# limuhit/360-Image-Compression

Hardware: AMD Instinct MI355X
Metric: ERP Mpixels/s enc+dec @512x1024 model-idx 3; bitstream bit-exact vs ref (higher is better)
Workload: dtype f32; 1 GPU; 192/GPU synthetic 512x1024 ERPs, model-idx 3 --ssim seed, latent+importance bitstreams, entropy enc+dec; streams=3, masks=smooth

## Files before the change

360-image-compression_amd/csrc/cconv4v6_dc.inc:

```
#define D6_GRID 256
#define D6_TAPE_BLOCKS 16
#define D6_TAPE_WAVES 6
#define D3_S0 (4 + C4_PS - 1)
#define D3_C0 2
#define D3_SP(h, w) ((h) + (w) - 1 + 2 * D3_S0)
#define D3_HP(h) ((h) + 2 * D3_C0)
struct Dc3Args {
    const float *x, *packed, *bias, *act, *residual;
    float *out;
    int ngroup, cout, hidden, H, W, npb, x_mod, N, psum, n_gb, n_gbv, nseg, pack0, gstep;
    int wblk;
    int nprod;
    int tape_c, tape_n, tape_total;
    unsigned tape_magic;
    unsigned tape_nw4[2];
};
struct Dc3Packed {
    const float *x, *packed, *bias, *act, *residual;
    float *out;
    unsigned w0;
    unsigned hw;
    int npb, x_mod, N;
    unsigned pg;
    int wblk, tape_n, tape_total;
// ... 38 lines not shown
        out[nwin++] = (unsigned)k | (unsigned)slo << 3 | (unsigned)shi << 9 | (unsigned)a0 << 15 | 1u << 21;
        pos = ((a0 + (shi - slo) + 4) / 4 + 1) * 4;
        slo = shi + 1;
        if (slo > hi) { slo = lo; ++k; }
    }
    return nwin;
}
__host__ __device__ __forceinline__ void dc6_wave_start(unsigned word, int lo, int hi, int h, int c, int wv, int &k, int &slo) {
    k = 0; slo = lo;
    if (wv == 0) return;
    const unsigned st = (word >> (9 * ((wv - 1) >> 1))) & 511u;
    k = st & 7; slo = st >> 3;
    if (!(wv & 1)) {
        unsigned pc[3];
        dc6_wave_pieces(lo, hi, h, c, k, slo, pc);
    }
}
#ifndef D6_STAGE_AT_END
#define D6_STAGE_AT_END 1
#endif
#ifndef D6_NB
#define D6_NB 2
#endif
#define D6_COLS 68
#define D6_QPR (D6_COLS / 4)
#define D6_ROWS (9 + C4_PS - 1)
#define D6_XQ(CIN) (4 * D6_ROWS * D6_QPR)
#define D6_XFL(CIN) (D6_XQ(CIN) * 4)

#define DPP_WAVE_SHL1 0x130
#define DPP_WAVE_SHR1 0x138
__device__ __forceinline__ float dpp_shl1(float v) {
    return __builtin_bit_cast(float, __builtin_amdgcn_update_dpp(0, __builtin_bit_cast(int, v), DPP_WAVE_SHL1, 0xf, 0xf, true));
}
__device__ __forceinline__ float dpp_shr1(float v) {
    return __builtin_bit_cast(float, __builtin_amdgcn_update_dpp(0, __builtin_bit_cast(int, v), DPP_WAVE_SHR1, 0xf, 0xf, true));
}

template <int CIN, int CLS, int XPLANE>
__device__ __forceinline__ void conv6_load(float *r0, const float *xl) {
    static_for<9>([&](auto dd) {
        constexpr int d = decltype(dd)::value, gid = CIN == 4 ? ((CLS - d) & 3) : 0, kmin = d > 4 ? d - 4 : 0, kmax = d < 4 ? d : 4;
        constexpr int k0 = kmax < 2 ? kmax : (kmin > 2 ? kmin : 2);
        if constexpr (CIN == 4 || (d & 3) == CLS) r0[d] = xl[gid * XPLANE + d * D6_COLS + k0];
    });
}
template <int CIN, int CLS, int D_LO, int D_HI>
__device__ __forceinline__ void conv6_diags(f32x4 *acc, const float *r0, float w0, float w1) {
    static_for<9>([&](auto dd) {
        constexpr int d = decltype(dd)::value, kmin = d > 4 ? d - 4 : 0, kmax = d < 4 ? d : 4;
        if constexpr (d >= D_LO && d <= D_HI && (CIN == 4 || (d & 3) == CLS)) {
            static_for<kmax - kmin + 1>([&](auto kk) {
                constexpr int kh = kmin + decltype(kk)::value, tap = 5 * kh + (d - kh), i = CIN == 4 ? tap : (tap - CLS) / 4;
                acc[i] = mfma4<i % 16>(i < 16 ? w0 : w1, r0[d], acc[i]);
            });
        }
    });
    __builtin_amdgcn_sched_barrier(0);
}
template <int CIN, int CLS>
__device__ __forceinline__ void conv6_align(f32x4 *acc) {
    static_for<9>([&](auto dd) {
        constexpr int d = decltype(dd)::value, kmin = d > 4 ? d - 4 : 0, kmax = d < 4 ? d : 4;
        constexpr int k0 = kmax < 2 ? kmax : (kmin > 2 ? kmin : 2);
        if constexpr (CIN == 4 || (d & 3) == CLS) {
            static_for<kmax - kmin + 1>([&](auto kk) {
                constexpr int kh = kmin + decltype(kk)::value, tap = 5 * kh + (d - kh), i = CIN == 4 ? tap : (tap - CLS) / 4, sh = kh - k0;
                static_for<(sh > 0 ? sh : -sh)>([&](auto) {
#pragma unroll
                    for (int r = 0; r < 4; ++r) acc[i][r] = sh > 0 ? dpp_shl1(acc[i][r]) : dpp_shr1(acc[i][r]);
                });
            });
        }
    });
}

struct W8 {
    float a0, a1, a2, a3, b0, b1, b2, b3;
    template <int H, int J> __device__ __forceinline__ float get() const {
        if constexpr (H == 0) return J == 0 ? a0 : (J == 1 ? a1 : (J == 2 ? a2 : a3));
        else return J == 0 ? b0 : (J == 1 ? b1 : (J == 2 ? b2 : b3));
    }
};

#define D6_SEG_STEP 60
#define D6_NSEG(h) ((h) <= 64 ? 1 : 1 + ((h) - 62 + D6_SEG_STEP - 1) / D6_SEG_STEP)
#ifdef DC6_STAMP
__device__ unsigned long long dc6_stamps[256 * 12 * 10];
#ifndef DC6_STAMP_CIN
#define DC6_STAMP_CIN 4
#endif
#define DC6_T(i) do { if constexpr (CIN == DC6_STAMP_CIN && !SEG) { const unsigned long long t_ = __builtin_amdgcn_s_memtime(); st[i] += t_ - t0; t0 = t_; } } while (0)
LIC360_API int lic360_dc6_stamps(unsigned long long *host_out, int clear) {
    if (host_out) HIP_TRY(hipMemcpyFromSymbol(host_out, HIP_SYMBOL(dc6_stamps), sizeof(dc6_stamps)));
    if (clear) { static unsigned long long z[256 * 12 * 10]; HIP_TRY(hipMemcpyToSymbol(HIP_SYMBOL(dc6_stamps), z, sizeof(z))); }
    return 0;
}
#else
#define DC6_T(i)
#endif
template <int CIN, int CLS, bool SEG, bool LAT = false, bool TAPE = false, bool LIST = false>
__device__ __forceinline__ void dc6_body(const Dc3Args &a, const Dc3Tape *tape, const uint4 *__restrict__ list, const int *__restrict__ lcnt, float *xs, float *comb,
                                         int (*trec)[16], int tid, int lane, int ps) {
    static_assert(!LIST || (TAPE && !SEG && !LAT), "list launches are throughput-mode launches of images of at most 64 rows");
    constexpr int XQ = D6_XQ(CIN), XFL = D6_XFL(CIN);
    static_assert(XQ <= C4_THREADS, "one quad slot per thread");
    constexpr int XPLANE = D6_ROWS * D6_COLS;
    const int H = a.H, W = a.W, G = a.ngroup, S = H + W - 1, HP = D3_HP(H);
    const int gs = a.gstep;
    constexpr int TCS = CIN == 1 ? 4 : 1;
    const long SKP = (long)D3_SP(H, W) * HP, tcs = 4 * SKP;
    f32x4 acc[NAcc<CIN>::value];
#ifdef DC6_STAMP
    unsigned long long st[10] = {0, 0, 0, 0, 0, 0, 0, 0, 0, 0}, t0 = __builtin_amdgcn_s_memtime();
    const unsigned long long t_entry = t0;
#endif
    const bool flat = gs == 1;
    const int xcd = flat ? 0 : blockIdx.x & 7, xstep = flat ? 1 : 8, wg_in_xcd = flat ? blockIdx.x : blockIdx.x >> 3;
    const int wgs_per_xcd = flat ? D6_GRID : (D6_GRID - xcd + 7) >> 3;
    auto nth_task = [&](int k) __attribute__((always_inline)) { return k * wgs_per_xcd + ((k & 1) ? wgs_per_xcd - 1 - wg_in_xcd : wg_in_xcd); };
    const int ns_x = flat ? a.N : (a.N - xcd + 7) >> 3;
    const int nseg = SEG ? a.nseg : 1;
    constexpr bool PACK = true;
    const bool pack_last = PACK && SEG && a.pack0 != 0;
    const int per_j = SEG ? ns_x * (nseg - 1) + (pack_last ? (ns_x + 1) >> 1 : ns_x) : 0;
    const int tape_c = TAPE ? a.tape_c : 0;
    const unsigned nw4[2] = {a.tape_nw4[0], a.tape_nw4[1]};
    auto blk_tasks = [&](int j) __attribute__((always_inline)) {
        return tape_c ? a.tape_n * (int)((nw4[(j >> 3) & 1] >> ((j & 7) * 4)) & 15u) : ns_x;
    };
    uint4 lrec = make_uint4(0u, 0u, 0u, 0u);
    if constexpr (LIST) {
        if (CLS == 0 && ps == 0) {
            int u = nth_task(lane);
            if (u > a.tape_total - 1) u = a.tape_total - 1;
            lrec = list[(long)xcd * a.tape_total + u];
        }
    }
    int n_my_ = 0;
    if constexpr (LIST) n_my_ = __builtin_amdgcn_readfirstlane(lcnt[xcd]);
    else if constexpr (SEG) n_my_ = per_j * a.n_gbv;
    else if (tape_c) n_my_ = a.tape_total;
    else n_my_ = ns_x * a.n_gbv;
    const int n_my = n_my_;
    int pk = -1, pq = 0;
    auto decode = [&](int u, int &g0, int &n, int &s0, int &seg, int &nb2, int &prb, int &packed) __attribute__((always_inline)) {
        nb2 = -1; prb = 0; packed = 0;
        if constexpr (LIST) {
            uint4 r;
            if (pk < 64) {
                r.x = (unsigned)__builtin_amdgcn_readlane((int)lrec.x, pk); r.y = (unsigned)__builtin_amdgcn_readlane((int)lrec.y, pk);
                r.z = (unsigned)__builtin_amdgcn_readlane((int)lrec.z, pk); r.w = (unsigned)__builtin_amdgcn_readlane((int)lrec.w, pk);
            } else r = list[(long)xcd * a.tape_total + u];
            g0 = (int)(r.x & 127u);
            n = (int)(r.x >> 10);
            s0 = a.psum - g0;
            seg = 0;
            if ((r.x >> 7) & 7u) { seg = (int)(r.y & 0x3fffffu); nb2 = (int)r.z; prb = (int)r.w; packed = 4; }
            packed |= (int)((r.y >> 22) & 7u) << 4;
        } else if constexpr (!SEG) {
            int j = 0, rem = u;
            for (; j < a.n_gbv - 1 && rem >= blk_tasks(j); ++j) rem -= blk_tasks(j);
            g0 = (a.n_gb - 1 - j) * gs;
            s0 = a.psum - g0;
            seg = 0;
            if (tape_c && (int)((nw4[(j >> 3) & 1] >> ((j & 7) * 4)) & 15u) < tape_c) {
                const int wv = a.tape_n == 1 ? rem : (int)__umulhi((unsigned)rem, a.tape_magic), tp = rem - wv * a.tape_n;
                n = xcd + 8 * tp * tape_c;
                int lo = 1 << 30, hi = -1;
#pragma unroll
                for (int q = 0; q < C4_PS; ++q) {
                    const int sq = s0 - q, l = sq >= W ? sq - W + 1 : 0, h2 = sq < H ? sq : H - 1;
                    if (g0 + q < G && sq >= 0 && sq < S) { lo = l < lo ? l : lo; hi = h2 > hi ? h2 : hi; }
                }
                int k, slo;
                dc6_wave_start(tape->s[j & (D6_TAPE_BLOCKS - 1)], lo, hi, H, tape_c, wv, k, slo);
                unsigned pc[3];
                dc6_wave_pieces(lo, hi, H, tape_c, k, slo, pc);
                seg = (int)pc[0]; nb2 = (int)pc[1]; prb = (int)pc[2];
                packed = 4;
            } else n = xcd + xstep * rem;
        } else {
            const int j = u / per_j, rem = u - j * per_j;
            g0 = (a.n_gb - 1 - j) * gs;
            s0 = a.psum - g0;
            if (pack_last && rem >= ns_x * (nseg - 1)) {
                seg = nseg - 1;
                n = xcd + 16 * (rem - ns_x * (nseg - 1));
                nb2 = n + 8;
                prb = H - 28;
                packed = 2;
            } else {
                seg = rem / ns_x;
                n = xcd + xstep * (rem - seg * ns_x);
            }
// ... 51 lines not shown
    auto issue_setup = [&]() __attribute__((always_inline)) {
        const int ig0 = rec(iq, 1), n = rec(iq, 2), is0 = rec(iq, 3), iseg = rec(iq, 4), inb = rec(iq, 5), iprb = rec(iq, 6);
        const int ipacked = rec(iq, 7) & 15;
        iL = steps_of(ig0);
        irl = ig0 + (C4_PS - 1) + 4 + a.hidden;
        const int irb = ipacked == 4 ? 0 : ((SEG && !ipacked) ? D6_SEG_STEP * iseg : iprb);
        ixn = (const char *)(a.x + (long)(n % a.x_mod) * G * CIN * SKP + (long)is0 * HP + irb);
        {
            const int qc = qa % D6_QPR;
            if (TAPE && ipacked == 4) {
                unsigned sh = 0u;
                bool cov = false;
                const unsigned stride8 = (unsigned)(8 * G * CIN * SKP * 4);
#pragma unroll
                for (int wi = 0; wi < 3; ++wi) {
                    const unsigned wd = (unsigned)(wi == 0 ? iseg : (wi == 1 ? inb : iprb));
                    const int k = wd & 7, slo = (wd >> 3) & 63, shi = (wd >> 9) & 63, a0 = (wd >> 15) & 63;
                    const bool in = (wd >> 21) != 0 && 4 * qc + 3 >= a0 && 4 * qc <= a0 + (shi - slo) + 4;
                    if (in) { sh = (unsigned)k * stride8 + (unsigned)((slo - a0) * 4); cov = true; }
                }
                t_off = cov ? offA + sh : 0u;
                t_off0 = cov ? offA0 + sh : 0u;
            } else if (SEG && PACK && ipacked) {
                const bool hb = qc > 8;
                const unsigned shift = hb ? (unsigned)(((long)((inb >= 0 ? inb : n) % a.x_mod) - (long)(n % a.x_mod)) * G * CIN * SKP * 4 - 9 * 16) : 0u;
                t_off = offA + shift;
                t_off0 = offA0 + shift;
            } else {
                const int lo = is0 - (gs - 1) - W + 1 - irb, hi = (is0 < H - 1 ? is0 : H - 1) - irb;
                const bool col_ok = qc >= ((lo > 0 ? lo : 0) >> 2) && qc <= ((hi + 4) >> 2);
                t_off = col_ok ? offA : 0u;
                t_off0 = col_ok ? offA0 : 0u;
            }
        }
        const int gg = ig0 + ps < G ? ig0 + ps : G - 1;
        iwp = (const char *)(a.packed + (((long)(n / a.npb) * G + gg) * a.wblk) * 1024);
    };
    if (!ivalid) return;
    issue_setup();
    const long tcs_b = tcs * 4;
    constexpr int WPSTEP = CIN == 4 ? 4096 : 8192;
    const char *px = ixn, *pw = iwp;
    auto issue_x2 = [&](f32x4 &ra, f32x4 &rb, int &tc0) __attribute__((always_inline)) -> const char * {
        const char *pwr = pw;
        tc0 = itc;
        unsigned oa, ob;
        if constexpr (CIN == 4) {
            oa = rowA < irl - itc ? t_off : t_off0;
            ob = rowA < irl - itc - 1 ? t_off : t_off0;
        } else {
            const int ta = itc + tcoA, tb = ta + TCS;
            oa = rowA < irl - ta ? t_off : t_off0;
            ob = rowA < irl - tb ? t_off : t_off0;
            if (ta >= G) oa = offP0;
            if (tb >= G) ob = offP0;
        }
        ra = *(const f32x4 *)(px + oa);
        rb = *(const f32x4 *)(px + (itc + TCS < G ? tcs_b : 0) + ob);
        if (ivalid) {
            px += 2 * tcs_b;
            pw += WPSTEP;
            itc += 2 * TCS;
            if (itc >= iL) {
                itc = 0;
                ++iq;
                ivalid = rec(iq, 0) != 0;
                if (ivalid) { issue_setup(); px = ixn; pw = iwp; }
                else { px -= 2 * tcs_b; pw -= WPSTEP; itc = tc0; }
            }
        }
        return pwr;
    };
    auto issue_w2 = [&](const char *p, int tc0, W8 &w) __attribute__((always_inline)) {
        (void)tc0;
        const f32x4 v = *(const f32x4 *)(p + offW);
        w.a0 = v[0]; w.a1 = v[1];
        if constexpr (CIN == 4) { w.b0 = v[2]; w.b1 = v[3]; }
        else {
            const f32x4 u = *(const f32x4 *)(p + offW + 4096);
            w.a2 = v[2]; w.a3 = v[3];
            w.b0 = u[0]; w.b1 = u[1]; w.b2 = u[2]; w.b3 = u[3];
        }
    };
    constexpr bool MIDST = D6_STAGE_AT_END == 0 || CIN == 1 || LAT || LIST;
    constexpr int NB = D6_NB, NBUF = 2 * D6_NB;
    static_assert(NB == 1 || NB == 2, "one or two double steps per barrier");
    f32x4 xa0 = {0.f, 0.f, 0.f, 0.f}, xb0 = xa0, xa1 = xa0, xb1 = xa0;
    W8 w0, w1;
    int tcw;
    { const char *p = issue_x2(xa0, xb0, tcw); issue_w2(p, tcw, w0); }
    { const char *p = issue_x2(xa1, xb1, tcw); issue_w2(p, tcw, w1); }
    if (hasA) { *(f32x4 *)ldsA = xa0; *(f32x4 *)(ldsA + XFL) = xb0; }
    int tcw_next, tcw_next2 = 0;
    const char *pw_next = issue_x2(xa0, xb0, tcw_next), *pw_next2 = nullptr;
    if constexpr (NB == 2) {
        if (hasA) { *(f32x4 *)(ldsA + 2 * XFL) = xa1; *(f32x4 *)(ldsA + 3 * XFL) = xb1; }
        pw_next2 = issue_x2(xa1, xb1, tcw_next2);
    }
    const f32x4 zero4 = {0.f, 0.f, 0.f, 0.f};
    int tq = 0, tc = 0, g0 = 0, n = 0, Lwg = 0, g = 0, s = 0, step = 0;
    bool glive = false, lane_ok = false;
    int n_lane = 0;
    float e_bias = 0.f, e_act = 0.f, e_res = 0.f;
    long e_oi = 0;
    const float *const act_p = a.act ? a.act : a.bias, *const res_p = a.residual ? a.residual : a.x;
    const float *const xl0 = xs + (C4_PS - 1 - ps) * D6_COLS + lane;
    auto task_setup = [&]() __attribute__((always_inline)) {
        g0 = rec(tq, 1); n = rec(tq, 2);
        const int s0 = rec(tq, 3), seg = rec(tq, 4), nb2 = rec(tq, 5), prb = rec(tq, 6);
        const int pk7 = rec(tq, 7), packed = pk7 & 15;
        Lwg = steps_of(g0);
        g = g0 + ps;
        s = s0 - ps;
        const int rb = packed == 4 ? 0 : ((SEG && !packed) ? D6_SEG_STEP * seg : prb);
        int row = rb + lane;
        n_lane = n;
        bool half_ok = true;
        if (TAPE && packed == 4) {
            half_ok = false;
            row = 0;
#pragma unroll
            for (int wi = 0; wi < 3; ++wi) {
                const unsigned wd = (unsigned)(wi == 0 ? seg : (wi == 1 ? nb2 : prb));
                const int k = wd & 7, slo = (wd >> 3) & 63, shi = (wd >> 9) & 63, a0 = (wd >> 15) & 63;
                if ((wd >> 21) != 0 && lane >= a0 && lane <= a0 + (shi - slo)) { half_ok = true; row = slo + lane - a0; n_lane = n + 8 * k; }
            }
        } else if (SEG && PACK && packed) {
            if (lane >= 36) { row = rb + lane - 36; n_lane = nb2 >= 0 ? nb2 : n; half_ok = nb2 >= 0; }
            else half_ok = lane < 28;
        }
        int sc;
        {
            int lo = s >= W ? s - W + 1 : 0, hi = s < H ? s : H - 1;
            const int segx = packed == 4 ? 0 : seg;
            if (lo < seg_lo(segx)) lo = seg_lo(segx);
            if (hi > seg_hi(segx)) hi = seg_hi(segx);
            glive = g < G && ps < gs && s >= 0 && s < S && lo <= hi && ((pk7 >> (4 + ps)) & 1) != 0;
            lane_ok = glive && half_ok && row >= lo && row <= hi;
            sc = s < 0 ? 0 : (s >= S ? S - 1 : s);
        }
#pragma unroll
        for (int i = 0; i < NAcc<CIN>::value; ++i) acc[i] = zero4;
        tc = 0;
        const int nout = G * a.cout, gc = g < G ? g : G - 1;
        const int o = gc * a.cout + (CLS < a.cout ? CLS : a.cout - 1), bid = (n / a.npb) * nout + o;
        e_oi = ((long)n_lane * nout + o) * SKP + (long)(sc + D3_S0) * HP + row + D3_C0;
        e_bias = a.bias[bid];
        e_act = act_p[bid];
        e_res = res_p[a.residual ? e_oi : 0];
    };
    auto epilogue = [&]() __attribute__((always_inline)) {
        conv6_align<CIN, CLS>(acc);
        const f32x4 part = tree4_eval<CIN, CLS>(acc);
        float *const cb = CIN == 1 ? comb + (tq & 1) * C4_COMB_FLOATS : comb;
#pragma unroll
        for (int r = 0; r < 4; ++r) cb[((ps * 4 + CLS) * 4 + r) * 64 + lane] = part[r];
        __syncthreads();
        const int r = CLS;
        if (lane_ok && r < a.cout) {
            const float f0 = cb[((ps * 4 + 0) * 4 + r) * 64 + lane], f1 = cb[((ps * 4 + 1) * 4 + r) * 64 + lane];
            const float f2 = cb[((ps * 4 + 2) * 4 + r) * 64 + lane], f3 = cb[((ps * 4 + 3) * 4 + r) * 64 + lane];
            float sv = ((f0 + f2) + (f1 + f3)) + e_bias;
            if (a.act) { if (sv < 0) sv = sv * e_act; }
            if (a.residual) sv = sv + e_res;
            a.out[e_oi] = sv;
        }
    };
    task_setup();
#define DC6_SUB(H_, J_, W_)                                                                     \
    if constexpr ((J_) < TCS) {                                                                 \
        constexpr int k = (H_) * TCS + (J_);                                                    \
        const int dl = dlim - k;                     \
        if (dl > 0 && tc + k < Lwg) {                                                           \
            float r0[9];                                                                        \
            conv6_load<CIN, CLS, XPLANE>(r0, xl + (H_) * XFL + (J_) * XPLANE);                  \
            __builtin_amdgcn_sched_barrier(0);                                                  \
            const float wa = W_.template get<(H_), (CIN == 4 ? 0 : (J_))>(), wb = W_.template get<(H_), 1>(); \
            conv6_diags<CIN, CLS, 0, 3>(acc, r0, wa, wb);                                       \
            if (dl > 4) conv6_diags<CIN, CLS, 4, 5>(acc, r0, wa, wb);                           \
            if (dl > 6) conv6_diags<CIN, CLS, 6, 8>(acc, r0, wa, wb);                           \
        }                                                                                       \
    }
#define DC6_HALF(H_, W_) DC6_SUB(H_, 0, W_) DC6_SUB(H_, 1, W_) DC6_SUB(H_, 2, W_) DC6_SUB(H_, 3, W_)
#define D6_STAGE_WRITE(XA_, XB_)                                                                \
        if (hasA) {                                                                             \
            float *q = ldsA + ((step + NB) & (NBUF - 1)) * (2 * XFL);                           \
            *(f32x4 *)q = XA_;                                                                  \
            *(f32x4 *)(q + XFL) = XB_;                                                          \
        }
#define D6_STAGE_BLOCK(XA_, XB_)                                                                \
        D6_STAGE_WRITE(XA_, XB_)                                                                \
        DC6_T(8);                        \
        pw_new = issue_x2(XA_, XB_, tcw_new);                                                   \
        __builtin_amdgcn_sched_barrier(0);
#define D6_STAGE_MID(XA_, XB_) if constexpr (MIDST) { D6_STAGE_BLOCK(XA_, XB_) }
#define D6_STAGE_END(XA_, XB_) if constexpr (!MIDST) { D6_STAGE_BLOCK(XA_, XB_) }
#define DC6_SUBSTEP(XA_, XB_, W_)                                                               \
    {                                                                                           \
        if (tc >= Lwg) {                                                                        \
            epilogue();                                                                         \
            ++tq;                                                                               \
            if (producer) produce();               \
            if (rec(tq, 0)) task_setup();                                                       \
            else { done = true; glive = false; Lwg = 0x7fffffff; }                              \
            DC6_ST7                                                                             \
        }                                                                                       \
        DC6_T(0);                                                                               \
        if (NB == 1 || (step & 1) == 0) __syncthreads();                                        \
        DC6_T(1);                                                                               \
        const int dlim = glive ? g + 4 + a.hidden - tc : 0;                                     \
        const float *xl = xl0 + (step & (NBUF - 1)) * (2 * XFL);                                \
        int tcw_new = 0;                                                                        \
        const char *pw_new = nullptr;                                                           \
        DC6_HALF(0, W_)                                                                         \
        DC6_T(2);                                                                               \
        D6_STAGE_MID(XA_, XB_)                                                                  \
        DC6_T(3);                                                                               \
        DC6_HALF(1, W_)                                                                         \
        D6_STAGE_END(XA_, XB_)                                                                  \
        DC6_T(4);                                                                               \
        issue_w2(pw_next, tcw_next, W_);                                                        \
        if constexpr (NB == 2) { pw_next = pw_next2; tcw_next = tcw_next2; pw_next2 = pw_new; tcw_next2 = tcw_new; } \
        else { pw_next = pw_new; tcw_next = tcw_new; }                                          \
        tc += 2 * TCS;                                                                          \
        ++step;                                                                                 \
        DC6_T(5);                                                                               \
        DC6_ST6                                                                                 \
    }
#ifdef DC6_STAMP
#define DC6_ST6 st[6] += 1;
#define DC6_ST7 st[7] += 1;
#else
#define DC6_ST6
#define DC6_ST7
#endif
    bool done = false;
    do {
        if constexpr (NB == 2) {
            DC6_SUBSTEP(xa0, xb0, w0)
            DC6_SUBSTEP(xa1, xb1, w1)
        } else {
            DC6_SUBSTEP(xa1, xb1, w0)
            DC6_SUBSTEP(xa0, xb0, w1)
        }
    } while (!done);
#ifdef DC6_STAMP
    if constexpr (CIN == DC6_STAMP_CIN && !SEG) {
        st[9] = __builtin_amdgcn_s_memtime() - t_entry;
        if (lane == 0) for (int i = 0; i < 10; ++i) dc6_stamps[((blockIdx.x & 255) * 12 + ps * 4 + CLS) * 10 + i] += st[i];
    }
#endif
#undef DC6_ST6
#undef DC6_ST7
#undef DC6_HALF
#undef DC6_SUB
#undef DC6_SUBSTEP
}

template <int CIN, bool SEG, bool LAT, bool TAPE, bool LIST = false>
__device__ __forceinline__ void dc6_kernel(const Dc3Packed &p, const Dc3Tape *tape, const uint4 *list = nullptr, const int *lcnt = nullptr) {
    __shared__ float xs[4 * D6_NB * D6_XFL(CIN)];
    __shared__ float comb[2 * C4_COMB_FLOATS];
    __shared__ int trec[8][16];
    const Dc3Args a = dc6_unpack(p);
    const int tid = threadIdx.x, lane = tid & 63;
    const int wave = __builtin_amdgcn_readfirstlane(tid >> 6), ps = wave >> 2, cls = wave & 3;
    switch (cls) {
        case 0: dc6_body<CIN, 0, SEG, LAT, TAPE, LIST>(a, tape, list, lcnt, xs, comb, trec, tid, lane, ps); break;
        case 1: dc6_body<CIN, 1, SEG, LAT, TAPE, LIST>(a, tape, list, lcnt, xs, comb, trec, tid, lane, ps); break;
        case 2: dc6_body<CIN, 2, SEG, LAT, TAPE, LIST>(a, tape, list, lcnt, xs, comb, trec, tid, lane, ps); break;
        default: dc6_body<CIN, 3, SEG, LAT, TAPE, LIST>(a, tape, list, lcnt, xs, comb, trec, tid, lane, ps); break;
    }
}
template <int CIN, bool SEG, bool LAT = false>
__global__ __launch_bounds__(C4_THREADS) void k_cconv4v6(Dc3Packed p) { dc6_kernel<CIN, SEG, LAT, false>(p, nullptr); }
template <int CIN>
__global__ __launch_bounds__(C4_THREADS) void k_cconv4v6t(Dc3Packed p, Dc3Tape tape) { dc6_kernel<CIN, false, false, true>(p, &tape); }
template <int CIN>
__global__ __launch_bounds__(C4_THREADS) void k_cconv4v6l(Dc3Packed p, const uint4 *list, const int *lcnt) { dc6_kernel<CIN, false, false, true, true>(p, nullptr, list, lcnt); }

static void dc6_build_tape(Dc3Args &a, Dc3Tape &tape, int h, int w, int cin, int n, int gs, bool nopack) {
    a.tape_c = 0; a.tape_n = 1; a.tape_total = 0; a.tape_magic = 0u; a.tape_nw4[0] = a.tape_nw4[1] = 0u;
    for (int j = 0; j < D6_TAPE_BLOCKS; ++j) tape.s[j] = 0u;
    const int S = h + w - 1, m = a.npb / 8;
    int c = 0;
    for (int t = D6_TAPE_WAVES; t >= 2 && !c; --t) if (m % t == 0) c = t;
    const bool ok = !nopack && a.nseg == 1 && gs == C4_PS && n % 8 == 0 && a.npb % 8 == 0 && c >= 2 && a.x_mod % (8 * c) == 0 && a.n_gbv <= D6_TAPE_BLOCKS &&
                    8.0 * c * a.ngroup * cin * (double)D3_SP(h, w) * D3_HP(h) * 4.0 < 4294967296.0;
    if (!ok) return;
    long old_tasks = 0, new_tasks = 0;
    int nws[D6_TAPE_BLOCKS];
    for (int j = 0; j < a.n_gbv; ++j) {
        const int gb = a.n_gb - 1 - j, s0 = a.psum - gb * C4_PS;
        int lo = 1 << 30, hi = -1;
        for (int q = 0; q < C4_PS; ++q) {
            const int sq = s0 - q;
            if (gb * C4_PS + q >= a.ngroup || sq < 0 || sq >= S) continue;
            const int l = sq >= w ? sq - w + 1 : 0, u = sq < h ? sq : h - 1;
            if (l < lo) lo = l;
            if (u > hi) hi = u;
        }
        int nw = 0, k = 0, slo = lo;
        unsigned starts = 0u;
        bool fits = hi >= 0;
        while (fits && k < c) {
            if (nw >= D6_TAPE_WAVES) { fits = false; break; }
            if (nw & 1) starts |= ((unsigned)k | (unsigned)slo << 3) << (9 * (nw >> 1));
            unsigned pc[3];
            if (dc6_wave_pieces(lo, hi, h, c, k, slo, pc) == 0) fits = false;
            ++nw;
        }
        if (!fits || nw >= c) {
            nw = c;
            starts = 0u;
        }
        tape.s[j] = starts;
        a.tape_nw4[j >> 3] |= (unsigned)nw << ((j & 7) * 4);
        nws[j] = nw;
        new_tasks += (long)nw * (m / c);
        old_tasks += m;
    }
    if (new_tasks > 0 && new_tasks < old_tasks) {
        a.tape_c = c;
        a.tape_n = n / 8 / c;
        a.tape_magic = (unsigned)((4294967296ull + a.tape_n - 1) / a.tape_n);
        for (int j = 0; j < a.n_gbv; ++j) a.tape_total += a.tape_n * nws[j];
    }
}

static bool dc6_schedule(Dc3Args &a, Dc3Tape &tape, int ngroup, int cin, int cout, int constrain, int n, int h, int w, int nb, int psum, int x_mod, bool nopack, int gstep_mode) {
    a.ngroup = ngroup; a.cout = cout; a.hidden = constrain == 5 ? 0 : 1; a.H = h; a.W = w; a.npb = n / nb; a.x_mod = x_mod; a.N = n;
    a.psum = psum;
    const int S = h + w - 1;
    int gb_lo = 1 << 30, gb_hi = -1;
    const int n_gb3 = (ngroup + C4_PS - 1) / C4_PS;
    const int gs = gstep_mode == 1 || (gstep_mode == 0 && (long)n * n_gb3 <= 128 && D6_NSEG(h) == 1) ? 1 : C4_PS;
    a.gstep = gs;
    {
        const int tcs2 = cin == 4 ? 2 : 8, lmin0 = (gs - 1) + 4 + a.hidden, lmin = lmin0 < ngroup ? lmin0 : ngroup;
        const int dmin = (lmin + tcs2 - 1) / tcs2, lead = (4 + dmin - 1) / dmin;
        a.nprod = lead + 2 < 6 ? lead + 2 : 6;
    }
    const int n_gb_all = (ngroup + gs - 1) / gs;
    for (int gb = 0; gb < n_gb_all; ++gb) {
        int s0 = psum - gb * gs;
        if (s0 - (gs - 1) >= S || s0 < 0) continue;
        if (gb < gb_lo) gb_lo = gb;
        if (gb > gb_hi) gb_hi = gb;
    }
    a.tape_c = 0; a.pack0 = 0;
    if (gb_hi < 0) return false;
    a.n_gb = gb_hi + 1;
    a.n_gbv = gb_hi - gb_lo + 1;
    a.nseg = D6_NSEG(h);
    dc6_build_tape(a, tape, h, w, cin, n, gs, nopack);
    if (a.nseg > 1 && a.npb % 16 == 0 && x_mod % 16 == 0 && !nopack && gs == C4_PS && h >= 28 && D6_SEG_STEP * (a.nseg - 1) + 2 >= h - 28 + 2) a.pack0 = 1;
    return true;
}

static int launch_cconv4v6_dc(hipStream_t stream, const lic360_conv_plan *p, const float *x, const float *packed4, const float *bias,
                              const float *act, const float *residual, float *out, int n, int h, int w, int nb, int psum, int x_mod, bool nopack,
                              int gstep_mode) {
    Dc3Args a;
    a.x = x; a.packed = packed4; a.wblk = conv4_wblk(p); a.bias = bias; a.act = act; a.residual = residual; a.out = out;
    ARG_CHECK(16.0 * p->ngroup * p->cin * (double)D3_SP(h, w) * D3_HP(h) * 4.0 < 4294967296.0);
    ARG_CHECK(h < 32768 && w < 32768 && D6_NSEG(h) <= 15 && p->ngroup <= 127 && p->cout <= 7 && psum >= 0 && psum < 65536);
    Dc3Tape tape;
    if (!dc6_schedule(a, tape, p->ngroup, p->cin, p->cout, p->constrain, n, h, w, nb, psum, x_mod, nopack, gstep_mode)) return 0;
    const int gs = a.gstep;
    const Dc3Packed pk = dc6_pack(a);
    if (a.nseg > 1) {
        if (p->cin == 4) hipLaunchKernelGGL((k_cconv4v6<4, true>), dim3(D6_GRID), dim3(C4_THREADS), 0, stream, pk);
        else hipLaunchKernelGGL((k_cconv4v6<1, true>), dim3(D6_GRID), dim3(C4_THREADS), 0, stream, pk);
    } else if (a.tape_c) {
        if (p->cin == 4) hipLaunchKernelGGL((k_cconv4v6t<4>), dim3(D6_GRID), dim3(C4_THREADS), 0, stream, pk, tape);
        else hipLaunchKernelGGL((k_cconv4v6t<1>), dim3(D6_GRID), dim3(C4_THREADS), 0, stream, pk, tape);
    } else if (p->cin == 4 && gs == 1) hipLaunchKernelGGL((k_cconv4v6<4, false, true>), dim3(D6_GRID), dim3(C4_THREADS), 0, stream, pk);
    else if (p->cin == 4) hipLaunchKernelGGL((k_cconv4v6<4, false>), dim3(D6_GRID), dim3(C4_THREADS), 0, stream, pk);
    else hipLaunchKernelGGL((k_cconv4v6<1, false>), dim3(D6_GRID), dim3(C4_THREADS), 0, stream, pk);
    LAUNCH_CHECK();
    return 0;
}

static int launch_cconv4v6_dc_list(hipStream_t stream, const lic360_conv_plan *p, const float *x, const float *packed4, const float *bias,
                                   const float *act, const float *residual, float *out, int n, int h, int w, int nb, int psum, int x_mod,
                                   const uint4 *list, const int *lcnt, int cap) {
    Dc3Args a;
    a.x = x; a.packed = packed4; a.wblk = conv4_wblk(p); a.bias = bias; a.act = act; a.residual = residual; a.out = out;
    ARG_CHECK(64.0 * p->ngroup * p->cin * (double)D3_SP(h, w) * D3_HP(h) * 4.0 < 4294967296.0);
    ARG_CHECK(h <= 64 && w < 32768 && p->ngroup <= 127 && p->cout <= 7 && psum >= 0 && psum < 65536 && p->cin == 4 && list && lcnt && cap > 0);
    ARG_CHECK(n % 8 == 0 && (n / nb) % 8 == 0 && x_mod == n);
    Dc3Tape tape;
    if (!dc6_schedule(a, tape, p->ngroup, p->cin, p->cout, p->constrain, n, h, w, nb, psum, x_mod, true, 3)) return 0;
    ARG_CHECK(a.gstep == C4_PS && a.nseg == 1);
    a.tape_c = 1;
    a.tape_total = cap;
    const Dc3Packed pk = dc6_pack(a);
    hipLaunchKernelGGL((k_cconv4v6l<4>), dim3(D6_GRID), dim3(C4_THREADS), 0, stream, pk, list, lcnt);
    LAUNCH_CHECK();
    return 0;
}

LIC360_API int lic360_dc4_tape_layout(int ngroup, int cin, int n, int nb, int h, int w, int psum, int x_mod, int *tape_c, int *n_blocks, int *blocks, int *nwaves, unsigned *windows) {
    ARG_CHECK(tape_c && n_blocks && blocks && nwaves && windows && ngroup > 0 && ngroup <= 64 && (cin == 1 || cin == 4) && n > 0 && nb > 0 && n % nb == 0 && h > 0 && w > 0 && x_mod > 0);
    Dc3Args a;
    *tape_c = 0; *n_blocks = 0;
    Dc3Tape tape;
    if (!dc6_schedule(a, tape, ngroup, cin, 4, cin == 4 ? 6 : 5, n, h, w, nb, psum, x_mod, false, 0)) return 0;
    *n_blocks = a.n_gbv < 24 ? a.n_gbv : 24;
    *tape_c = a.tape_c;
    for (int j = 0; j < 24 * 6 * 3; ++j) windows[j] = 0u;
    for (int j = 0; j < a.n_gbv && j < 24; ++j) {
        blocks[j] = (a.n_gb - 1 - j) * a.gstep;
        nwaves[j] = a.tape_c ? (int)((a.tape_nw4[(j >> 3) & 1] >> ((j & 7) * 4)) & 15u) : 0;
        if (!a.tape_c || nwaves[j] >= a.tape_c) continue;
        int lo = 1 << 30, hi = -1;
        for (int q = 0; q < C4_PS; ++q) {
            const int sq = psum - blocks[j] - q;
            if (blocks[j] + q >= ngroup || sq < 0 || sq >= h + w - 1) continue;
            const int l = sq >= w ? sq - w + 1 : 0, u = sq < h ? sq : h - 1;
            if (l < lo) lo = l;
            if (u > hi) hi = u;
        }
        for (int t = 0; t < nwaves[j]; ++t) {
            int k, slo;
            dc6_wave_start(tape.s[j], lo, hi, h, a.tape_c, t, k, slo);
            dc6_wave_pieces(lo, hi, h, a.tape_c, k, slo, &windows[(j * 6 + t) * 3]);
        }
    }
    return 0;
}
```

360-image-compression_amd/csrc/codec_fused.hip:

```cpp
#include "common.h"
#include "conv_plan.h"
#include "ac_core.h"
#include "lic360_exact_math.h"
#include "gmm_tables.h"
#include "need.h"
#include <vector>
#include <cstring>
#include <algorithm>
#include <thread>
#include <atomic>
#include <memory>
#include <immintrin.h>

struct AcDevState {
    uint32_t low, high, code;
    int nacc, error, pad;
    long pos;
    unsigned long long acc;
};

struct PlanDeleter { void operator()(lic360_conv_plan *p) const { lic360_conv_plan_destroy(p); } };
using PlanPtr = std::unique_ptr<lic360_conv_plan, PlanDeleter>;
static int make_plan(PlanPtr &out, int channel, int ngroup, int nout, int ksz, int constrain) {
    lic360_conv_plan *p = nullptr;
// ... 1536 lines not shown
    ARG_CHECK(c);
    c->prof = on != 0;
    for (int k = 0; k < PROF_NCLS; ++k) c->n_ev[k] = 0;
    return 0;
}
LIC360_API const char *lic360_codec_profile_classes(void) { return PROF_NAMES; }

LIC360_API int lic360_codec_profile_read(lic360_codec *c, int n, double *ms, long *launches) {
    ARG_CHECK(c && ms && launches && n >= PROF_NCLS);
    for (int k = 0; k < PROF_NCLS; ++k) {
        double acc = 0;
        const size_t cnt = c->n_ev[k];
        for (size_t i = 0; i + 1 < cnt; i += 2) {
            HIP_TRY(hipEventSynchronize(c->ev[k][i + 1]));
            float t = 0;
            HIP_TRY(hipEventElapsedTime(&t, c->ev[k][i], c->ev[k][i + 1]));
            acc += t;
        }
        ms[k] = acc;
        launches[k] = (long)(cnt / 2);
        c->n_ev[k] = 0;
    }
    return 0;
}

LIC360_API int lic360_codec_skip_stats(lic360_codec *c, int enable, unsigned long long *out, int *skip_active_out) {
    ARG_CHECK(c);
    if (skip_active_out) *skip_active_out = c->skip ? 1 + (c->dcl.list ? 1 : 0) : 0;
    if (!c->skip) { if (out) memset(out, 0, 2 * NEED_LAYERS * NEED_STAT_G * sizeof(unsigned long long)); return 0; }
    if (enable >= 0) c->stats_on = enable != 0;
    if (out) {
        HIP_TRY(hipDeviceSynchronize());
        HIP_TRY(hipMemcpy(out, c->stats, 2 * NEED_LAYERS * NEED_STAT_G * sizeof(unsigned long long), hipMemcpyDeviceToHost));
        HIP_TRY(hipMemset(c->stats, 0, 2 * NEED_LAYERS * NEED_STAT_G * sizeof(unsigned long long)));
    }
    return 0;
}
__global__ void k_fill_enc(float *buf, long planes, int H, int W, int hp, int wp, int off, float v) {
    GRID_STRIDE(i, planes * H * W) {
        const int x = (int)(i % W), y = (int)((i / W) % H);
        buf[(i / ((long)H * W)) * hp * wp + e_cell(y, x, wp, off)] = v;
    }
}
__global__ void k_fill_dec(float *buf, long planes, int H, int W, int sk_rows, int sk_pitch, int row0, int col0, float v) {
    GRID_STRIDE(i, planes * H * W) {
        const int x = (int)(i % W), y = (int)((i / W) % H);
        buf[(i / ((long)H * W)) * sk_rows * sk_pitch + (long)(y + x + row0) * sk_pitch + y + col0] = v;
    }
}
LIC360_API int lic360_codec_debug_fill(void *stream, lic360_codec *c, float value) {
    ARG_CHECK(c && value == value && value - value == 0.0f);
    hipStream_t s = (hipStream_t)stream;
    const long B = c->maxB, G = c->G;
    for (int i = 0; i < 3; ++i) {
        hipLaunchKernelGGL(k_fill_enc, dim3(lic360_blocks(3 * B * 4 * G * c->HW, 4)), dim3(256), 0, s, c->e_buf[i], 3 * B * 4 * G, c->H, c->W, c->e_hp, c->e_wp, c->e_off, value);
        LAUNCH_CHECK();
    }
    for (int i = 0; i < 11; ++i) {
        hipLaunchKernelGGL(k_fill_dec, dim3(lic360_blocks(3 * B * 4 * G * c->HW, 4)), dim3(256), 0, s, c->d_act[i], 3 * B * 4 * G, c->H, c->W, c->sk_rows, c->sk_pitch, c->sk_row0, c->sk_col0, value);
        LAUNCH_CHECK();
    }
    hipLaunchKernelGGL(k_fill_dec, dim3(lic360_blocks(3 * B * 3 * G * c->HW, 4)), dim3(256), 0, s, c->d_y, 3 * B * 3 * G, c->H, c->W, c->sk_rows, c->sk_pitch, c->sk_row0, c->sk_col0, value);
    LAUNCH_CHECK();
    return 0;
}
LIC360_API int lic360_codec_debug_lists(lic360_codec *c, int which, void *host_out, long bytes, int *cap_out) {
    ARG_CHECK(c && host_out && bytes >= 0 && which >= 0 && which <= 4 && c->skip);
    HIP_TRY(hipDeviceSynchronize());
    const void *src = nullptr;
    long have = 0;
    if (which == 0) { src = c->need; have = (long)c->maxB * NEED_LAYERS * c->HW; }
    else if (which == 1) { src = c->ecl.cnt; have = NEED_LAYERS * 8 * 4L; }
    else if (which == 2) { src = c->ecl.list; have = (long)NEED_LAYERS * 8 * c->ecl.cap * 4; }
    else if (which == 3) { src = c->dcl.cnt; have = c->dcl.list ? (long)NEED_LAYERS * c->P * 8 * 4 : 0; }
    else { src = c->dcl.list; have = c->dcl.list ? (long)NEED_LAYERS * c->P * 8 * c->dcl.cap * 16 : 0; }
    if (cap_out) *cap_out = which <= 2 ? c->ecl.cap : c->dcl.cap;
    ARG_CHECK(src && bytes <= have);
    HIP_TRY(hipMemcpy(host_out, src, (size_t)bytes, hipMemcpyDeviceToHost));
    return 0;
}

LIC360_API const char *lic360_codec_kernel_names(void) {
    return "ec_first=k_cconv16<1, false>;ec_hidden=k_cconv16s+k_cconv16<4, false>;ec_last=k_cconv16<4, true>;"
           "dc_first=k_cconv4v6<1, false, false>+k_cconv4v6t<1>;"
           "dc_hidden=k_cconv4v6l<4>+k_cconv4v6t<4>+k_cconv4v6<4, false, false>+k_cconv4v6<4, false, true>;"
           "dc_last=k_cconv4v6l<4>+k_cconv4v6t<4>+k_cconv4v6<4, false, false>+k_cconv4v6<4, false, true>;"
           "imp_ec=k_cconv144<1, false, 2>;imp_dc=k_cconv144<1, true, 2>";
}
```

Baseline: 59.56 Mpixel/s.

## Compute three nets per task in first-layer decoder context conv to share input loads

Adds a three-net variant of the dc6 context-convolution body for the first (CIN=1) layer. Each task now accumulates outputs for all three nets (streams) from one staged input tile, loading each net's weights at its own offset, and the epilogue writes three outputs. This removes the repeated input staging and scheduling across three separate per-net tasks. The cost is more accumulator registers (three times as many), a tripled combine buffer in shared memory, an extra barrier per epilogue, and a changed weight-prefetch pattern, all of which may lower occupancy.

```diff
diff --git a/360-image-compression_amd/csrc/cconv4v6_dc.inc b/360-image-compression_amd/csrc/cconv4v6_dc.inc
--- a/360-image-compression_amd/csrc/cconv4v6_dc.inc
+++ b/360-image-compression_amd/csrc/cconv4v6_dc.inc
@@ -144,6 +144,14 @@
         else return J == 0 ? b0 : (J == 1 ? b1 : (J == 2 ? b2 : b3));
     }
 };
+template <int CIN, int CLS, int D_LO, int D_HI, int NETS, int H, int J>
+__device__ __forceinline__ void conv6_diags_nets(f32x4 *acc, const float *r0, const W8 *w) {
+    constexpr int NA = NAcc<CIN>::value;
+    static_for<NETS>([&](auto qq) {
+        constexpr int q = decltype(qq)::value;
+        conv6_diags<CIN, CLS, D_LO, D_HI>(acc + q * NA, r0, w[q].template get<H, (CIN == 4 ? 0 : J)>(), w[q].template get<H, 1>());
+    });
+}
 
 #define D6_SEG_STEP 60
 #define D6_NSEG(h) ((h) <= 64 ? 1 : 1 + ((h) - 62 + D6_SEG_STEP - 1) / D6_SEG_STEP)
@@ -161,10 +169,11 @@
 #else
 #define DC6_T(i)
 #endif
-template <int CIN, int CLS, bool SEG, bool LAT = false, bool TAPE = false, bool LIST = false>
+template <int CIN, int CLS, bool SEG, bool LAT = false, bool TAPE = false, bool LIST = false, int NETS = 1>
 __device__ __forceinline__ void dc6_body(const Dc3Args &a, const Dc3Tape *tape, const uint4 *__restrict__ list, const int *__restrict__ lcnt, float *xs, float *comb,
                                          int (*trec)[16], int tid, int lane, int ps) {
     static_assert(!LIST || (TAPE && !SEG && !LAT), "list launches are throughput-mode launches of images of at most 64 rows");
+    static_assert(NETS == 1 || (NETS == 3 && CIN == 1 && !SEG && !LAT && !LIST), "three nets per task: the first layer's throughput-mode launches");
     constexpr int XQ = D6_XQ(CIN), XFL = D6_XFL(CIN);
     static_assert(XQ <= C4_THREADS, "one quad slot per thread");
     constexpr int XPLANE = D6_ROWS * D6_COLS;
@@ -172,7 +181,8 @@
     const int gs = a.gstep;
     constexpr int TCS = CIN == 1 ? 4 : 1;
     const long SKP = (long)D3_SP(H, W) * HP, tcs = 4 * SKP;
-    f32x4 acc[NAcc<CIN>::value];
+    constexpr int NA = NAcc<CIN>::value;
+    f32x4 acc[NETS * NA];
 #ifdef DC6_STAMP
     unsigned long long st[10] = {0, 0, 0, 0, 0, 0, 0, 0, 0, 0}, t0 = __builtin_amdgcn_s_memtime();
     const unsigned long long t_entry = t0;
@@ -390,14 +400,30 @@
             w.b0 = u[0]; w.b1 = u[1]; w.b2 = u[2]; w.b3 = u[3];
         }
     };
+    const long wnet = NETS > 1 ? (long)G * a.wblk * 4096 : 0;
+    auto issue_wn = [&](const char *p, int tc0, W8 *w) __attribute__((always_inline)) {
+#pragma unroll
+        for (int q = 0; q < NETS; ++q) issue_w2(p + q * wnet, tc0, w[q]);
+    };
+    const char *pw_next1 = nullptr;
+    auto issue_wh = [&](auto hh, W8 *w) __attribute__((always_inline)) {
+        constexpr int h = decltype(hh)::value;
+#pragma unroll
+        for (int q = 0; q < NETS; ++q) {
+            const f32x4 v = *(const f32x4 *)(pw_next1 + q * wnet + offW + h * 4096);
+            if constexpr (h == 0) { w[q].a0 = v[0]; w[q].a1 = v[1]; w[q].a2 = v[2]; w[q].a3 = v[3]; }
+            else { w[q].b0 = v[0]; w[q].b1 = v[1]; w[q].b2 = v[2]; w[q].b3 = v[3]; }
+        }
+    };
     constexpr bool MIDST = D6_STAGE_AT_END == 0 || CIN == 1 || LAT || LIST;
     constexpr int NB = D6_NB, NBUF = 2 * D6_NB;
     static_assert(NB == 1 || NB == 2, "one or two double steps per barrier");
+    static_assert(NETS == 1 || NB == 2, "the three-net form is written for two double steps per barrier");
     f32x4 xa0 = {0.f, 0.f, 0.f, 0.f}, xb0 = xa0, xa1 = xa0, xb1 = xa0;
-    W8 w0, w1;
+    W8 w0[NETS], w1[NETS];
     int tcw;
-    { const char *p = issue_x2(xa0, xb0, tcw); issue_w2(p, tcw, w0); }
-    { const char *p = issue_x2(xa1, xb1, tcw); issue_w2(p, tcw, w1); }
+    { const char *p = issue_x2(xa0, xb0, tcw); issue_wn(p, tcw, w0); }
+    { const char *p = issue_x2(xa1, xb1, tcw); if constexpr (NETS > 1) pw_next1 = p; else issue_wn(p, tcw, w1); }
     if (hasA) { *(f32x4 *)ldsA = xa0; *(f32x4 *)(ldsA + XFL) = xb0; }
     int tcw_next, tcw_next2 = 0;
     const char *pw_next = issue_x2(xa0, xb0, tcw_next), *pw_next2 = nullptr;
@@ -409,8 +435,9 @@
     int tq = 0, tc = 0, g0 = 0, n = 0, Lwg = 0, g = 0, s = 0, step = 0;
     bool glive = false, lane_ok = false;
     int n_lane = 0;
-    float e_bias = 0.f, e_act = 0.f, e_res = 0.f;
+    float e_bias[NETS], e_act[NETS], e_res[NETS];
     long e_oi = 0;
+    const long e_onet = NETS > 1 ? (long)a.N * G * a.cout * SKP : 0;
     const float *const act_p = a.act ? a.act : a.bias, *const res_p = a.residual ? a.residual : a.x;
     const float *const xl0 = xs + (C4_PS - 1 - ps) * D6_COLS + lane;
     auto task_setup = [&]() __attribute__((always_inline)) {
@@ -448,31 +475,49 @@
             sc = s < 0 ? 0 : (s >= S ? S - 1 : s);
         }
 #pragma unroll
-        for (int i = 0; i < NAcc<CIN>::value; ++i) acc[i] = zero4;
+        for (int i = 0; i < NETS * NA; ++i) acc[i] = zero4;
         tc = 0;
         const int nout = G * a.cout, gc = g < G ? g : G - 1;
         const int o = gc * a.cout + (CLS < a.cout ? CLS : a.cout - 1), bid = (n / a.npb) * nout + o;
         e_oi = ((long)n_lane * nout + o) * SKP + (long)(sc + D3_S0) * HP + row + D3_C0;
-        e_bias = a.bias[bid];
-        e_act = act_p[bid];
-        e_res = res_p[a.residual ? e_oi : 0];
+        if constexpr (NETS == 1) {
+            e_bias[0] = a.bias[bid];
+            e_act[0] = act_p[bid];
+            e_res[0] = res_p[a.residual ? e_oi : 0];
+        } else {
+#pragma unroll
+            for (int q = 0; q < NETS; ++q) {
+                e_bias[q] = a.bias[bid + q * nout];
+                e_act[q] = act_p[bid + q * nout];
+                e_res[q] = res_p[a.residual ? e_oi + q * e_onet : 0];
+            }
+        }
     };
     auto epilogue = [&]() __attribute__((always_inline)) {
-        conv6_align<CIN, CLS>(acc);
-        const f32x4 part = tree4_eval<CIN, CLS>(acc);
-        float *const cb = CIN == 1 ? comb + (tq & 1) * C4_COMB_FLOATS : comb;
-#pragma unroll
-        for (int r = 0; r < 4; ++r) cb[((ps * 4 + CLS) * 4 + r) * 64 + lane] = part[r];
+        static_for<NETS>([&](auto qq) {
+            constexpr int q = decltype(qq)::value;
+            conv6_align<CIN, CLS>(acc + q * NA);
+            const f32x4 part = tree4_eval<CIN, CLS>(acc + q * NA);
+            float *const cb = NETS > 1 ? comb + q * C4_COMB_FLOATS : (CIN == 1 ? comb + (tq & 1) * C4_COMB_FLOATS : comb);
+#pragma unroll
+            for (int r = 0; r < 4; ++r) cb[((ps * 4 + CLS) * 4 + r) * 64 + lane] = part[r];
+        });
         __syncthreads();
         const int r = CLS;
         if (lane_ok && r < a.cout) {
-            const float f0 = cb[((ps * 4 + 0) * 4 + r) * 64 + lane], f1 = cb[((ps * 4 + 1) * 4 + r) * 64 + lane];
-            const float f2 = cb[((ps * 4 + 2) * 4 + r) * 64 + lane], f3 = cb[((ps * 4 + 3) * 4 + r) * 64 + lane];
-            float sv = ((f0 + f2) + (f1 + f3)) + e_bias;
-            if (a.act) { if (sv < 0) sv = sv * e_act; }
-            if (a.residual) sv = sv + e_res;
-            a.out[e_oi] = sv;
-        }
+            static_for<NETS>([&](auto qq) {
+                constexpr int q = decltype(qq)::value;
+                const float *const cb = NETS > 1 ? comb + q * C4_COMB_FLOATS : (CIN == 1 ? comb + (tq & 1) * C4_COMB_FLOATS : comb);
+                const float f0 = cb[((ps * 4 + 0) * 4 + r) * 64 + lane], f1 = cb[((ps * 4 + 1) * 4 + r) * 64 + lane];
+                const float f2 = cb[((ps * 4 + 2) * 4 + r) * 64 + lane], f3 = cb[((ps * 4 + 3) * 4 + r) * 64 + lane];
+                float sv = ((f0 + f2) + (f1 + f3)) + e_bias[q];
+                if (a.act) { if (sv < 0) sv = sv * e_act[q]; }
+                if (a.residual) sv = sv + e_res[q];
+                if constexpr (q == 0) a.out[e_oi] = sv;
+                else a.out[e_oi + q * e_onet] = sv;
+            });
+        }
+        if constexpr (NETS > 1) __syncthreads();
     };
     task_setup();
 #define DC6_SUB(H_, J_, W_)                                                                     \
@@ -483,10 +528,9 @@
             float r0[9];                                                                        \
             conv6_load<CIN, CLS, XPLANE>(r0, xl + (H_) * XFL + (J_) * XPLANE);                  \
             __builtin_amdgcn_sched_barrier(0);                                                  \
-            const float wa = W_.template get<(H_), (CIN == 4 ? 0 : (J_))>(), wb = W_.template get<(H_), 1>(); \
-            conv6_diags<CIN, CLS, 0, 3>(acc, r0, wa, wb);                                       \
-            if (dl > 4) conv6_diags<CIN, CLS, 4, 5>(acc, r0, wa, wb);                           \
-            if (dl > 6) conv6_diags<CIN, CLS, 6, 8>(acc, r0, wa, wb);                           \
+            conv6_diags_nets<CIN, CLS, 0, 3, NETS, (H_), (J_)>(acc, r0, W_);                    \
+            if (dl > 4) conv6_diags_nets<CIN, CLS, 4, 5, NETS, (H_), (J_)>(acc, r0, W_);        \
+            if (dl > 6) conv6_diags_nets<CIN, CLS, 6, 8, NETS, (H_), (J_)>(acc, r0, W_);        \
         }                                                                                       \
     }
 #define DC6_HALF(H_, W_) DC6_SUB(H_, 0, W_) DC6_SUB(H_, 1, W_) DC6_SUB(H_, 2, W_) DC6_SUB(H_, 3, W_)
@@ -522,12 +566,14 @@
         const char *pw_new = nullptr;                                                           \
         DC6_HALF(0, W_)                                                                         \
         DC6_T(2);                                                                               \
+        if constexpr (NETS > 1) issue_wh(IC<0>{}, W_);                                          \
         D6_STAGE_MID(XA_, XB_)                                                                  \
         DC6_T(3);                                                                               \
         DC6_HALF(1, W_)                                                                         \
         D6_STAGE_END(XA_, XB_)                                                                  \
         DC6_T(4);                                                                               \
-        issue_w2(pw_next, tcw_next, W_);                                                        \
+        if constexpr (NETS > 1) { issue_wh(IC<1>{}, W_); pw_next1 = pw_next; }                  \
+        else issue_wn(pw_next, tcw_next, W_);                                                   \
         if constexpr (NB == 2) { pw_next = pw_next2; tcw_next = tcw_next2; pw_next2 = pw_new; tcw_next2 = tcw_new; } \
         else { pw_next = pw_new; tcw_next = tcw_new; }                                          \
         tc += 2 * TCS;                                                                          \
@@ -544,7 +590,10 @@
 #endif
     bool done = false;
     do {
-        if constexpr (NB == 2) {
+        if constexpr (NB == 2 && NETS > 1) {
+            DC6_SUBSTEP(xa0, xb0, w0)
+            DC6_SUBSTEP(xa1, xb1, w0)
+        } else if constexpr (NB == 2) {
             DC6_SUBSTEP(xa0, xb0, w0)
             DC6_SUBSTEP(xa1, xb1, w1)
         } else {
@@ -565,19 +614,19 @@
 #undef DC6_SUBSTEP
 }
 
-template <int CIN, bool SEG, bool LAT, bool TAPE, bool LIST = false>
+template <int CIN, bool SEG, bool LAT, bool TAPE, bool LIST = false, int NETS = 1>
 __device__ __forceinline__ void dc6_kernel(const Dc3Packed &p, const Dc3Tape *tape, const uint4 *list = nullptr, const int *lcnt = nullptr) {
     __shared__ float xs[4 * D6_NB * D6_XFL(CIN)];
-    __shared__ float comb[2 * C4_COMB_FLOATS];
+    __shared__ float comb[(NETS > 1 ? NETS : 2) * C4_COMB_FLOATS];
     __shared__ int trec[8][16];
     const Dc3Args a = dc6_unpack(p);
     const int tid = threadIdx.x, lane = tid & 63;
     const int wave = __builtin_amdgcn_readfirstlane(tid >> 6), ps = wave >> 2, cls = wave & 3;
     switch (cls) {
-        case 0: dc6_body<CIN, 0, SEG, LAT, TAPE, LIST>(a, tape, list, lcnt, xs, comb, trec, tid, lane, ps); break;
-        case 1: dc6_body<CIN, 1, SEG, LAT, TAPE, LIST>(a, tape, list, lcnt, xs, comb, trec, tid, lane, ps); break;
-        case 2: dc6_body<CIN, 2, SEG, LAT, TAPE, LIST>(a, tape, list, lcnt, xs, comb, trec, tid, lane, ps); break;
-        default: dc6_body<CIN, 3, SEG, LAT, TAPE, LIST>(a, tape, list, lcnt, xs, comb, trec, tid, lane, ps); break;
+        case 0: dc6_body<CIN, 0, SEG, LAT, TAPE, LIST, NETS>(a, tape, list, lcnt, xs, comb, trec, tid, lane, ps); break;
+        case 1: dc6_body<CIN, 1, SEG, LAT, TAPE, LIST, NETS>(a, tape, list, lcnt, xs, comb, trec, tid, lane, ps); break;
+        case 2: dc6_body<CIN, 2, SEG, LAT, TAPE, LIST, NETS>(a, tape, list, lcnt, xs, comb, trec, tid, lane, ps); break;
+        default: dc6_body<CIN, 3, SEG, LAT, TAPE, LIST, NETS>(a, tape, list, lcnt, xs, comb, trec, tid, lane, ps); break;
     }
 }
 template <int CIN, bool SEG, bool LAT = false>
@@ -586,6 +635,8 @@
 __global__ __launch_bounds__(C4_THREADS) void k_cconv4v6t(Dc3Packed p, Dc3Tape tape) { dc6_kernel<CIN, false, false, true>(p, &tape); }
 template <int CIN>
 __global__ __launch_bounds__(C4_THREADS) void k_cconv4v6l(Dc3Packed p, const uint4 *list, const int *lcnt) { dc6_kernel<CIN, false, false, true, true>(p, nullptr, list, lcnt); }
+__global__ __launch_bounds__(C4_THREADS) void k_cconv4v6x3(Dc3Packed p) { dc6_kernel<1, false, false, false, false, 3>(p, nullptr); }
+__global__ __launch_bounds__(C4_THREADS) void k_cconv4v6x3t(Dc3Packed p, Dc3Tape tape) { dc6_kernel<1, false, false, true, false, 3>(p, &tape); }
 
 static void dc6_build_tape(Dc3Args &a, Dc3Tape &tape, int h, int w, int cin, int n, int gs, bool nopack) {
     a.tape_c = 0; a.tape_n = 1; a.tape_total = 0; a.tape_magic = 0u; a.tape_nw4[0] = a.tape_nw4[1] = 0u;
@@ -676,6 +727,14 @@
     Dc3Tape tape;
     if (!dc6_schedule(a, tape, p->ngroup, p->cin, p->cout, p->constrain, n, h, w, nb, psum, x_mod, nopack, gstep_mode)) return 0;
     const int gs = a.gstep;
+    if (p->cin == 1 && nb == 3 && x_mod * 3 == n && a.nseg == 1 && gs == C4_PS) {
+        if (!dc6_schedule(a, tape, p->ngroup, 1, p->cout, p->constrain, x_mod, h, w, 1, psum, x_mod, nopack, 3)) return 0;
+        const Dc3Packed pk = dc6_pack(a);
+        if (a.tape_c) hipLaunchKernelGGL(k_cconv4v6x3t, dim3(D6_GRID), dim3(C4_THREADS), 0, stream, pk, tape);
+        else hipLaunchKernelGGL(k_cconv4v6x3, dim3(D6_GRID), dim3(C4_THREADS), 0, stream, pk);
+        LAUNCH_CHECK();
+        return 0;
+    }
     const Dc3Packed pk = dc6_pack(a);
     if (a.nseg > 1) {
         if (p->cin == 4) hipLaunchKernelGGL((k_cconv4v6<4, true>), dim3(D6_GRID), dim3(C4_THREADS), 0, stream, pk);
diff --git a/360-image-compression_amd/csrc/codec_fused.hip b/360-image-compression_amd/csrc/codec_fused.hip
--- a/360-image-compression_amd/csrc/codec_fused.hip
+++ b/360-image-compression_amd/csrc/codec_fused.hip
@@ -1642,7 +1642,7 @@
 
 LIC360_API const char *lic360_codec_kernel_names(void) {
     return "ec_first=k_cconv16<1, false>;ec_hidden=k_cconv16s+k_cconv16<4, false>;ec_last=k_cconv16<4, true>;"
-           "dc_first=k_cconv4v6<1, false, false>+k_cconv4v6t<1>;"
+           "dc_first=k_cconv4v6x3t+k_cconv4v6x3;"
            "dc_hidden=k_cconv4v6l<4>+k_cconv4v6t<4>+k_cconv4v6<4, false, false>+k_cconv4v6<4, false, true>;"
            "dc_last=k_cconv4v6l<4>+k_cconv4v6t<4>+k_cconv4v6<4, false, false>+k_cconv4v6<4, false, true>;"
            "imp_ec=k_cconv144<1, false, 2>;imp_dc=k_cconv144<1, true, 2>";
```

New measurement: 60.12 Mpixel/s, median of 6. No clear change (+0.9%).
